# lastz/lastz

Hardware: AMD Instinct MI355X
Metric: Gbp-of-target aligned/sec (whole job, --nogapped HSP path, both strands) (higher is better)
Workload: dtype s32

## Files before the change

include/lzgpu.h:

```cpp
#ifndef LZGPU_H
#define LZGPU_H
#include <stdint.h>
#include <stddef.h>

#ifdef __cplusplus
extern "C" {
#endif

#define LZGPU_MAX_PARTS   16
#define LZGPU_MAX_PROBES  128

#define LZGPU_ERR_NO_DEVICE   (-1)
#define LZGPU_ERR_HIP         (-2)
#define LZGPU_ERR_OOM         (-3)
#define LZGPU_ERR_ARG         (-4)
#define LZGPU_ERR_STATE       (-5)

#define LZGPU_NH_SEED          1
#define LZGPU_NH_SCORE_CLASSES 2
#define LZGPU_NH_HITS_OVERFLOW 3
#define LZGPU_NH_HSP_OVERFLOW  4
#define LZGPU_NH_SIZE          5
#define LZGPU_NH_IDENTICAL     6
#define LZGPU_NH_UNSUPPORTED   7
// ... 158 lines not shown
int lzgpu_reduce_to_chain(const lz_chain_args* a, const lz_segment* segs, uint32_t n, uint32_t** kept, uint32_t* n_kept, int32_t* best);
int lzgpu_reduce_to_chain_batch(const lz_chain_args* a, const lz_segment* const* segs, const uint32_t* n, uint32_t k,
                                uint32_t** kept, uint32_t* n_kept, int32_t* best);

typedef struct lz_counters {
    uint64_t words;
    uint64_t raw_hits;
    uint64_t extensions;
    uint64_t bp_extended;
    uint64_t hsps;
    uint64_t dp_cells;
    uint64_t gapped_extensions;
    uint64_t anchors_extended;
    uint64_t truncated_extensions;
    uint64_t dp_rows;
} lz_counters;
void lzgpu_counters_reset(void);
int  lzgpu_counters_get(lz_counters* out);

void lzgpu_profile_enable(int enable);
void lzgpu_profile_reset(void);
int  lzgpu_profile_get(int n, const char** name, uint64_t* launches, double* total_ms);

int lzgpu_set_hit_capacity(uint64_t max_hits_per_chunk);
int lzgpu_set_hsp_capacity(uint64_t max_candidate_hsps);
int lzgpu_set_dp_slot(uint32_t first_try_traceback_bytes_per_dp);
int lzgpu_set_dp_window(uint32_t max_anchors_speculated_per_round);
int lzgpu_dp_longest(uint64_t out[4], int reset);

int lzgpu_set_bucket_owner(uint32_t n_owners, uint32_t owner);
int lzgpu_last_scan_mode(void);
int lzgpu_set_scan_mode(int min_mode);
int lzgpu_last_hsp_order(uint64_t* out , uint64_t n);

#ifdef __cplusplus
}
#endif
#endif
```

lastz_amd/build.py:

```python
import os
import subprocess
import sys

HERE = os.path.dirname(os.path.abspath(__file__))
CSRC = os.environ.get("LZGPU_CSRC") or os.path.join(HERE, "csrc")
OUT = os.path.join(HERE, "liblzgpu.so")
SOURCES = ["lzgpu_api.hip", "seq_kernels.hip", "table_kernels.hip", "limit_kernels.hip", "mask_kernels.hip", "enum_kernels.hip", "scan_kernels.hip", "exact_kernels.hip", "mismatch_kernels.hip", "filter_kernels.hip", "settle_kernels.hip", "dp_kernels.hip", "dp_kernels_narrow.hip", "window_kernels.hip", "lz_share.hip", "lz_host.cpp", "lz_gapped_host.cpp", "lz_dp_pieces.cpp", "lz_chain_host.cpp"]
FLAGS = ["--offload-arch=gfx950", "-O3", "-std=c++17", "-fPIC", "-Wall", "-Wno-unused-result"] + os.environ.get("LZGPU_CXXFLAGS", "").split()


def _stale(obj, srcs):
    if not os.path.exists(obj):
        return True
    t = os.path.getmtime(obj)
    return any(os.path.getmtime(s) > t for s in srcs)


def build(force=False, verbose=False):
    hipcc = os.environ.get("HIPCC", "/opt/rocm/bin/hipcc")
    tag = os.environ.get("LZGPU_BUILD_TAG", "")
    out = OUT if not tag else os.path.join(HERE, "liblzgpu_%s.so" % tag)
    objdir = os.path.join(HERE, "build" if not tag else "build_" + tag)
    os.makedirs(objdir, exist_ok=True)
    headers = [os.path.join(CSRC, f) for f in os.listdir(CSRC) if f.endswith((".hpp", ".h", ".inc"))]
    headers.append(os.path.join(HERE, "..", "include", "lzgpu.h"))
    objs = []
    procs = []
    for src in SOURCES:
        sp = os.path.join(CSRC, src)
        obj = os.path.join(objdir, src + ".o")
        objs.append(obj)
        if force or _stale(obj, [sp] + headers):
            flags = FLAGS if src.endswith(".hip") else ["-x", "c++"] + [f for f in FLAGS if not f.startswith("--offload")]
            cmd = [hipcc] + flags + ["-c", sp, "-o", obj]
            if verbose:
                print(" ".join(cmd))
            procs.append((src, subprocess.Popen(cmd)))
    for src, p in procs:
        if p.wait() != 0:
            raise RuntimeError(f"hipcc failed on {src}")
# ... 11 lines not shown
```

lastz_amd/csrc/lz_ctx.hpp:

```cpp
#pragma once
#include <hip/hip_runtime.h>
#include <string>
#include <vector>
#include <map>
#include <mutex>
#include "lz_common.hpp"
#include "lz_settings.hpp"
#include "../../include/lzgpu.h"

struct DevBuf {
    void*  p = nullptr;
    size_t cap = 0;
    int ensure(size_t bytes);
    void release();
    template <class T> T* as() const { return (T*)p; }
};

struct KernelTimer {
    struct Pending { int id; hipEvent_t a, b; hipStream_t s; };
    bool enabled = false;
    std::vector<std::string> names;
    std::vector<uint64_t> launches;
    std::vector<double> ms;
    std::vector<Pending> pending;
// ... 60 lines not shown
    DevBuf wctx;
    u64 wctx_gen = 0; uint64_t wctx_code_key = 0;

    std::map<int, SeqSlot> queries;
#define LZ_TEMP_SLOT_B3 (-1000)
    std::mutex slots_m;

    DevBuf cnt, off, pk;
    DevBuf wiv, wsk, wsv;
    DevBuf blk_start;
    std::vector<u64> blk_start_host;
    u32 blk_shift = 0, blk_count = 1;
    u64* pinned = nullptr; size_t pinned_words = 0;
    DevBuf bins;
    DevBuf keys;
    DevBuf keys2;
    DevBuf filter_keep, filter_counts, filter_bases;
    DevBuf bin_base;
    DevBuf hist, hist_part, run_addr;
    DevBuf summ, scan_tasks, scan_ntasks;
    DevBuf lut;
    DevBuf sort_tmp, scan_tmp;
    DevBuf diag_end;
    DevBuf score_tab;
    std::vector<s32> score_sub;
    u8 rowc[256] = { 0 }, colc[256] = { 0 };
    std::vector<s32> lut_m4; s32 lut_xdrop = -1;
    DevBuf cls_t, cls_q, cls_tmp;
    DevBuf win_tab;
    DevBuf match_tmp;
    DevBuf hsp_out, hsp_count;
    DevBuf hsp_mc;
    DevBuf dev_counters;
    DevBuf tb_keys, tb_vals, tb_keys2, tb_vals2;
    DevBuf mask_bits, mask_ranges;
    struct DpBufs { DevBuf jobs, ids, res, tab, tb, rows, ops, ops_off, ops_out, pieces, rings, sel_jobs, sel_res, problems; } dp;
    DevBuf win_jobs, win_scratch, win_out, win_count;
    bool win_attr_set = false;
    bool settle_attr_set = false;
    bool settle_exact_attr_set = false;
    bool settle_mismatch_attr_set = false;
    u64 dp_longest[4] = { 0, 0, 0, 0 };
    u32 dp_slot_tb = 8u << 20;
    u32 dp_window = 0;
    u32 n_owners = 1, owner = 0;
    bool filter_on = false;
    lz_hit_filter filter = {};
    u64 filter_dropped = 0;
    LzSelfDev self = {};
    DevBuf self_sep;
    std::vector<u64> last_order;
    int min_scan_mode = 0;
    int last_scan_mode = -1;
    u64 hit_capacity = (1ull << 31);
    u64 hsp_capacity = (1ull << 24);

    lz_counters counters = {};
    std::mutex counters_m;
    KernelTimer timer;
    KernelTimer dp_timer;

    void release_device_memory()
    {
        DevBuf* all[] = { &wstart, &wpos, &full_wstart, &full_wpos, &wctx, &cnt, &off, &pk, &wiv, &wsk, &wsv, &blk_start, &bins, &keys, &keys2, &filter_keep, &filter_counts, &filter_bases, &bin_base, &hist, &hist_part, &run_addr,
                          &summ, &scan_tasks, &scan_ntasks, &lut, &sort_tmp, &scan_tmp, &diag_end, &score_tab, &cls_t, &cls_q, &cls_tmp, &win_tab, &match_tmp,
                          &hsp_out, &hsp_count, &hsp_mc, &dev_counters, &tb_keys, &tb_vals, &tb_keys2, &tb_vals2, &mask_bits, &mask_ranges, &self_sep,
                          &dp.jobs, &dp.ids, &dp.res, &dp.tab, &dp.tb, &dp.rows, &dp.ops, &dp.ops_off, &dp.ops_out, &dp.pieces, &dp.rings, &dp.sel_jobs, &dp.sel_res, &dp.problems,
                          &win_jobs, &win_scratch, &win_out, &win_count };
        for (DevBuf* b : all) b->release();
        target.release();
        for (auto& kv : queries) kv.second.release();
        queries.clear();
        if (pinned) (void)hipHostFree(pinned);
        pinned = nullptr; pinned_words = 0;
        have_table = false; wctx_gen = 0; wctx_code_key = 0; limit = 0; full_num_words = 0;
        score_sub.clear(); lut_m4.clear(); lut_xdrop = -1;
        win_attr_set = false; settle_attr_set = false; settle_exact_attr_set = false; settle_mismatch_attr_set = false;
    }
};

LzCtx& lz_ctx();
int lz_bind_thread();
int lz_fail(int code, const char* fmt, ...);
#define LZ_HIP(expr) do { hipError_t _e = (expr); if (_e != hipSuccess) \
    return lz_fail(LZGPU_ERR_HIP, "%s:%d %s -> %s", __FILE__, __LINE__, #expr, hipGetErrorString(_e)); } while (0)

struct LzChunk; struct LzLutParams; struct LzExactParams; struct LzMismatchParams; struct LzFilterParams;
#include "lz_tile_runs.hpp"
int lzk_encode(LzCtx& c, const u8* raw, u8* code, u32 len, const u8* cls256_dev, hipStream_t st = nullptr, KernelTimer* timer = nullptr);
int lzk_pack_nibbles(LzCtx& c, const u8* code_alloc, u8* nib, size_t nbytes);
int lzk_pack2(LzCtx& c, const u8* code_base, const u8* raw_base, u32 len, u8* two, u8* spc, u32 nmask, u32* flags256);
int lzk_overlap32(LzCtx& c, const u8* src, u8* dst, size_t nblocks);
int lzk_table_build(LzCtx& c);
int lzk_table_export(LzCtx& c, u32* last_dev, u32* prev_dev, u32 prev_entries);
int lzk_wctx_build(LzCtx& c);
void lz_limit_lift(LzCtx& c);
int lzk_table_limit(LzCtx& c, u32 limit);
int lzk_table_count_distribution(LzCtx& c, std::vector<u32>& count, std::vector<u32>& words);
int lzk_table_mask(LzCtx& c, const lz_interval* iv, u32 n, u32 tlen);
int lzk_count_hits(LzCtx& c, const u8* qcode, u32 lo, u32 hi);
int lzk_scan_counts(LzCtx& c, u32 n);
int lzk_sample_offsets(LzCtx& c, u32 n, u32 stride, u32 ns);
int lzk_fill_hits(LzCtx& c, u32 lo, const LzChunk& ch, u32 n);
int lzk_scan_reserve(LzCtx& c, int mode, u64 max_n);
int lzk_scan_hits(LzCtx& c, int mode, const LzExtendParams& P, const LzLutParams& Q, u64 n);
int lzk_fused_reserve(LzCtx& c, u64 max_n);
int lzk_scan_fused(LzCtx& c, u32 lo, const LzChunk& ch, u32 n, const LzExtendParams& P, const LzLutParams& Q);
int lzk_partition(LzCtx& c, bool tagged, u64 n);
int lzk_hist_scan(LzCtx& c, u64 n);
int lzk_settle(LzCtx& c, const LzExtendParams& P, u64 n, u32 out_cap);
int lzk_hsp_match_counts(LzCtx& c, u32 n_rec, const SeqSlot& q);
int lzk_settle_exact(LzCtx& c, const LzExactParams& P, u64 n, u32 out_cap);
int lzk_settle_mismatch(LzCtx& c, const LzMismatchParams& P, u64 n, u32 out_cap);
int lzk_scan_exact(LzCtx& c, const LzExactParams& P, u64 n);
int lzk_scan_mismatch(LzCtx& c, const LzMismatchParams& P, u64 n);
int lzk_filter_reserve(LzCtx& c, u64 max_n);
int lzk_filter_hits(LzCtx& c, const LzFilterParams& F, u64 n, u64* n_kept);
```

lastz_amd/csrc/lz_settings.hpp:

```cpp
#pragma once
#include <stdlib.h>
#include <string>

struct LzSettings {
    bool hostprof;
    bool gaps;
    std::string timer_only;
    int scan_mode;
    unsigned long long hit_capacity;
    bool fused_scan;
    unsigned task_region_cap;
    unsigned dp_horizon;
    unsigned helper_min_anchors;
    unsigned helpers;
    unsigned batch_threads;
    unsigned chain_threads;
};

struct LzDpSwitches {
    int narrow, repl;
    std::string dump;
    bool prof;
    unsigned window;
};

namespace lz_env {
inline int      flag01(const char* e) { return e ? e[0] == '1' : -1; }
inline unsigned positive(const char* e, unsigned unset) { const int v = e ? atoi(e) : 0; return v > 0 ? (unsigned)v : unset; }
}

inline LzSettings lz_settings_read()
{
    using namespace lz_env;
    LzSettings s;
    s.hostprof = getenv("LZGPU_HOSTPROF") != nullptr;
    s.gaps = getenv("LZGPU_GAPS") != nullptr;
    { const char* e = getenv("LZGPU_TIMER_ONLY"); s.timer_only = e ? e : ""; }
    { const char* e = getenv("LZGPU_SCAN_MODE"); const int v = e ? atoi(e) : -1; s.scan_mode = v >= 0 && v <= 2 ? v : -1; }
    { const char* e = getenv("LZGPU_HIT_CAPACITY"); const long long v = e ? atoll(e) : 0; s.hit_capacity = v >= 1024 && v <= (1ll << 31) ? (unsigned long long)v : 0; }
    { const char* e = getenv("LZGPU_FUSED_SCAN"); s.fused_scan = !(e && atoi(e) == 0); }
    s.task_region_cap = positive(getenv("LZGPU_TASK_REGION_CAP"), 0);
    { const char* e = getenv("LZGPU_DP_HORIZON"); s.dp_horizon = (unsigned)(e ? atoi(e) : 0); }
    { const char* e = getenv("LZGPU_HELPER_MIN_ANCHORS"); s.helper_min_anchors = (unsigned)(e ? atoi(e) : 20000); }
    s.helpers = positive(getenv("LZGPU_HELPERS"), 0);
    s.batch_threads = positive(getenv("LZGPU_BATCH_THREADS"), 64);
    s.chain_threads = positive(getenv("LZGPU_CHAIN_THREADS"), 16);
    return s;
}
inline const LzSettings& lz_settings() { static const LzSettings s = lz_settings_read(); return s; }

inline LzDpSwitches lz_dp_switches()
{
    using namespace lz_env;
    LzDpSwitches d;
    d.narrow = flag01(getenv("LZGPU_DP_NARROW"));
    d.repl = flag01(getenv("LZGPU_DP_REPL"));
    { const char* e = getenv("LZGPU_DPDUMP"); d.dump = e ? e : ""; }
    d.prof = getenv("LZGPU_DPPROF") != nullptr;
    d.window = positive(getenv("LZGPU_DP_WINDOW"), 0);
    return d;
}
```

lastz_amd/csrc/lzgpu_api.hip:

```cpp
#include <hip/hip_runtime.h>
#include <stdarg.h>
#include <stdio.h>
#include <stdlib.h>
#include <string.h>
#include <math.h>
#include <algorithm>
#include <mutex>
#include <thread>
#include <atomic>
#include "lz_ctx.hpp"
#include "lz_host.hpp"
#include "lz_lut.hpp"
#include "lz_exact.hpp"
#include "lz_mismatch.hpp"
#include "lz_filter.hpp"


static LzCtx g_ctx;
void lz_phase_clocks_print();
LzCtx& lz_ctx() { return g_ctx; }

static thread_local std::string t_last_error, t_last_error_out;
static std::mutex g_err_m;
int lz_fail(int code, const char* fmt, ...)
{
    char buf[512];
    va_list ap; va_start(ap, fmt); vsnprintf(buf, sizeof(buf), fmt, ap); va_end(ap);
    t_last_error = buf;
    std::lock_guard<std::mutex> lk(g_err_m);
    g_ctx.last_error = buf;
    return code;
}

int DevBuf::ensure(size_t bytes)
{
    if (bytes <= cap && p) return 0;
    const bool prof = lz_settings().hostprof;
    const auto t0 = std::chrono::steady_clock::now();
    const size_t old = cap;
    if (p) { (void)hipFree(p); p = nullptr; cap = 0; }
    const auto t1 = std::chrono::steady_clock::now();
    size_t want = bytes < 256 ? 256 : bytes;
    if (want >= (64u << 20)) {
        size_t step = (size_t)1 << 22;
        while (step * 32 <= want) step <<= 1;
        want = (want + step - 1) / step * step;
    }
    hipError_t e = hipMalloc(&p, want);
// ... 73 lines not shown
    return t_last_error_out.c_str();
}

extern "C" int lzgpu_probe(void)
{
    int n = 0;
    if (hipGetDeviceCount(&n) != hipSuccess || n <= 0) return lz_fail(LZGPU_ERR_NO_DEVICE, "no HIP device visible");
    hipDeviceProp_t prop;
    if (hipGetDeviceProperties(&prop, 0) != hipSuccess) return lz_fail(LZGPU_ERR_NO_DEVICE, "hipGetDeviceProperties failed");
    if (strncmp(prop.gcnArchName, "gfx950", 6) != 0)
        return lz_fail(LZGPU_ERR_NO_DEVICE, "device 0 is %s, this library is built for gfx950 only", prop.gcnArchName);
    return 0;
}

static int lz_init_locked(int device_index)
{
    if (g_ctx.inited && (device_index < 0 || device_index == g_ctx.device)) return 0;
    if (g_ctx.inited) return lz_fail(LZGPU_ERR_STATE, "already bound to device %d", g_ctx.device);
    int rc = lzgpu_probe();
    if (rc) return rc;
    if (device_index < 0) {
        const char* lr = getenv("LOCAL_RANK");
        device_index = lr ? atoi(lr) : 0;
        int n = 0; (void)hipGetDeviceCount(&n);
        if (n > 0) device_index %= n;
    }
    LZ_HIP(hipSetDevice(device_index));
    { hipDeviceProp_t prop; if (hipGetDeviceProperties(&prop, device_index) == hipSuccess && prop.multiProcessorCount > 0) g_ctx.num_cus = prop.multiProcessorCount; }
    LZ_HIP(hipStreamCreateWithFlags(&g_ctx.stream, hipStreamNonBlocking));
    LZ_HIP(hipStreamCreateWithFlags(&g_ctx.dp_stream, hipStreamNonBlocking));
    const LzSettings& S = lz_settings();
    if (S.scan_mode >= 0) g_ctx.min_scan_mode = S.scan_mode;
    if (S.hit_capacity) g_ctx.hit_capacity = S.hit_capacity;
    g_ctx.device = device_index;
    g_ctx.inited = true;
    return 0;
}

static std::mutex g_init_mutex;
static std::atomic<int> g_async_state{0};
static void lz_wait_async() { while (g_async_state.load(std::memory_order_acquire) == 1) std::this_thread::yield(); }
extern "C" void lzgpu_init_async(int device_index)
{
    int expect = 0;
    if (!g_async_state.compare_exchange_strong(expect, 1)) return;
    atexit(lz_wait_async);
    std::thread([device_index]() {
        { std::lock_guard<std::mutex> lk(g_init_mutex); (void)lz_init_locked(device_index); }
        g_async_state.store(2, std::memory_order_release);
    }).detach();
}
extern "C" int lzgpu_init(int device_index)
{
    lz_wait_async();
    std::lock_guard<std::mutex> lk(g_init_mutex);
    const int rc = lz_init_locked(device_index);
    if (!rc) LZ_HIP(hipSetDevice(g_ctx.device));
    return rc;
}
extern "C" int lzgpu_device_index(void) { return g_ctx.inited ? g_ctx.device : -1; }

extern "C" void lzgpu_shutdown(void)
{
    LzCtx& c = g_ctx;
    if (!c.inited) return;
    (void)hipSetDevice(c.device);
// ... 673 lines not shown
    if ((rc = ss_filter(c, s, nh))) return rc;
    if (nh == 0) return 0;
    std::vector<u64> hk(nh);
    LZ_HIP(hipMemcpyAsync(hk.data(), c.keys.p, (size_t)nh * 8, hipMemcpyDeviceToHost, c.stream));
    LZ_HIP(hipStreamSynchronize(c.stream));
    for (u64 k : hk) { u32 p2 = (u32)k; s.plain.push_back({ p2 + (u32)(k >> 32), p2, s.L, 0 }); }
    return 0;
}

static int ss_finish(LzCtx& c, SeedSearch& s, lz_hsp** out, uint64_t* n_out)
{
    const lz_search_args* a = s.a;
    int rc;
    u64 hc[3] = { 0, 0, 0 }; u32 n_rec = 0;
    LZ_HIP(hipMemcpyAsync(hc, c.dev_counters.p, 24, hipMemcpyDeviceToHost, c.stream));
    LZ_HIP(hipMemcpyAsync(&n_rec, c.hsp_count.p, 4, hipMemcpyDeviceToHost, c.stream));
    LZ_HIP(hipStreamSynchronize(c.stream));
    g_hp.lap(4, "wait for GPU");
    const bool extend = s.extend();
    const s32 K = s.exact() ? 0 : a->hsp_threshold;
    const int entropic = s.exact() ? 0 : a->entropic;
    const bool gpu_counts = extend && n_rec > 0 && n_rec <= s.out_cap;
    if (gpu_counts) {
        if ((rc = c.hsp_mc.ensure((size_t)n_rec * 20))) return rc;
        if ((rc = lzk_hsp_match_counts(c, n_rec, *s.qs))) return rc;
    }
    c.timer.resolve();
    { std::lock_guard<std::mutex> lk(c.counters_m);
      c.counters.words += hc[2]; c.counters.raw_hits += s.total_hits;
      c.counters.extensions += hc[0]; c.counters.bp_extended += hc[1]; }
    if (!extend) return lz_hsps_out(s.plain, out, n_out);
    if (n_rec > s.out_cap) return LZGPU_NH_HSP_OVERFLOW;

    std::vector<LzHspRec> recs(n_rec);
    std::vector<u32> mc;
    if (n_rec) LZ_HIP(hipMemcpyAsync(recs.data(), c.hsp_out.p, (size_t)n_rec * sizeof(LzHspRec), hipMemcpyDeviceToHost, c.stream));
    if (gpu_counts) { mc.resize((size_t)n_rec * 5); LZ_HIP(hipMemcpyAsync(mc.data(), c.hsp_mc.p, (size_t)n_rec * 20, hipMemcpyDeviceToHost, c.stream)); }
    LZ_HIP(hipStreamSynchronize(c.stream));
    c.timer.resolve();
    g_hp.lap(5, "copy candidates");
    std::vector<lz_hsp> fin;
    if ((rc = lzh_finish_hsps(recs.data(), n_rec, c.target.host.data(), s.qhost, c.seed, c.geom.char_to_bits,
                              K, entropic, fin, gpu_counts ? mc.data() : nullptr, &c.last_order)))
        return lz_fail(rc, "internal: candidate HSP is not on a seed hit");
    if ((rc = lz_hsps_out(fin, out, n_out))) return rc;
    { std::lock_guard<std::mutex> lk(c.counters_m); c.counters.hsps += fin.size(); }
    g_hp.lap(6, "host finish (order+entropy)");
    return 0;
}

static int filter_check(LzCtx& c, const int8_t* match_bits)
{
    if (!c.filter_on) return 0;
    const lz_hit_filter& f = c.filter;
    const u32 L = (u32)c.seed.length;
    if (f.positions == 0 || (L < 32 && (f.positions >> L) != 0)) return lz_fail(LZGPU_ERR_ARG, "hit filter: positions %08x of a seed of length %u", f.positions, L);
    if (f.min_matches < 0 || f.min_matches > __builtin_popcount(f.positions))
        return lz_fail(LZGPU_ERR_ARG, "hit filter: %d matches of %d positions", (int)f.min_matches, __builtin_popcount(f.positions));
    if (match_bits && memcmp(match_bits, f.match_bits, 256) != 0)
        return lz_fail(LZGPU_ERR_ARG, "hit filter: the search's match_bits differ from the filter's (a slot holds one set of match codes)");
    if (c.n_owners > 1) return LZGPU_NH_UNSUPPORTED;
    return 0;
}

static int seed_search(const lz_search_args* a, lz_hsp** out, uint64_t* n_out, const int8_t* match_bits = nullptr, u32 mismatches = 0)
{
    LzCtx& c = g_ctx;
    SeedSearch s; s.a = a; s.match_bits = match_bits; s.mismatches = mismatches;
    int rc;
    c.filter_dropped = 0;
    if ((rc = filter_check(c, match_bits))) return rc;
    s.filtered = c.filter_on;
    g_hp.start();
    if ((rc = ss_query(c, s))) return rc;
    if ((rc = ss_classes(c, s))) return rc;
    if (s.qs->len < s.L) return 0;
    if ((rc = ss_count(c, s))) return rc;
    if ((rc = ss_plan(c, s))) return rc;
    if ((rc = ss_scan_mode(c, s))) return rc;
    if ((rc = ss_reserve(c, s))) return rc;
    for (const LzChunk& ch : s.chunks) if ((rc = s.exact() ? ss_chunk_exact(c, s, ch) : a->extend ? ss_chunk(c, s, ch) : ss_chunk_plain(c, s, ch))) return rc;
    g_hp.lap(3, "chunk loop launches");
    return ss_finish(c, s, out, n_out);
}

extern "C" int lzgpu_seed_hit_search(const lz_search_args* a, lz_hsp** out, uint64_t* n_out)
{
    int rc = search_enter(a && out && n_out && a->sub, out, n_out);
    return rc ? rc : seed_search(a, out, n_out);
}

extern "C" int lzgpu_seed_hit_search_exact(const lz_search_args* a, const int8_t match_bits[256], lz_hsp** out, uint64_t* n_out)
{
    int rc = search_enter(a && match_bits && out && n_out, out, n_out); if (rc) return rc;
    if (g_ctx.n_owners > 1) return LZGPU_NH_UNSUPPORTED;
    return seed_search(a, out, n_out, match_bits);
}

extern "C" int lzgpu_seed_hit_search_mismatch(const lz_search_args* a, const int8_t match_bits[256], int32_t max_mismatches, lz_hsp** out, uint64_t* n_out)
{
    int rc = search_enter(a && match_bits && out && n_out, out, n_out); if (rc) return rc;
    if (max_mismatches < 1 || max_mismatches > (int32_t)LZ_MM_MAX) return lz_fail(LZGPU_ERR_ARG, "in seed_hit_search_mismatch(), %d mismatches (1..%u)", (int)max_mismatches, LZ_MM_MAX);
    if (a->hsp_threshold < 1) return lz_fail(LZGPU_ERR_ARG, "in seed_hit_search_mismatch(), length %d", (int)a->hsp_threshold);
// ... 120 lines not shown
    return 0;
}
extern "C" int lzgpu_set_hit_capacity(uint64_t n)
{
    if (n < 1024 || n > (1ull << 31)) return LZGPU_ERR_ARG;
    g_ctx.hit_capacity = n; return 0;
}
extern "C" int lzgpu_set_bucket_owner(uint32_t n_owners, uint32_t owner)
{
    if (n_owners < 1 || n_owners > LZ_DIAG_SIZE || owner >= n_owners) return LZGPU_ERR_ARG;
    g_ctx.n_owners = n_owners; g_ctx.owner = owner;
    return 0;
}
extern "C" int lzgpu_set_hit_filter(const lz_hit_filter* f)
{
    g_ctx.filter_on = f != nullptr;
    if (f) g_ctx.filter = *f;
    return 0;
}
extern "C" int lzgpu_last_filter_dropped(uint64_t* dropped)
{
    if (!dropped) return LZGPU_ERR_ARG;
    *dropped = g_ctx.filter_dropped;
    return 0;
}
extern "C" int lzgpu_last_hsp_order(uint64_t* out, uint64_t n)
{
    if (!out || 2 * n != g_ctx.last_order.size()) return LZGPU_ERR_ARG;
    memcpy(out, g_ctx.last_order.data(), g_ctx.last_order.size() * 8);
    return 0;
}
extern "C" int lzgpu_last_scan_mode(void) { return g_ctx.last_scan_mode; }
extern "C" int lzgpu_set_scan_mode(int min_mode) { if (min_mode < 0 || min_mode > 2) return LZGPU_ERR_ARG; g_ctx.min_scan_mode = min_mode; return 0; }
extern "C" int lzgpu_set_hsp_capacity(uint64_t n) { if (n < 16) return LZGPU_ERR_ARG; g_ctx.hsp_capacity = n; return 0; }
```

lastz_amd/lzgpu.py:

```python
import ctypes as C
import os
import numpy as np

_HERE = os.path.dirname(os.path.abspath(__file__))
LIB_PATH = os.environ.get("LZGPU_LIB") or os.path.join(_HERE, "liblzgpu.so")

MAX_PARTS, MAX_PROBES = 16, 128

NH_REASONS = {1: "SEED", 2: "SCORE_CLASSES", 3: "HITS_OVERFLOW", 4: "HSP_OVERFLOW", 5: "SIZE",
              6: "IDENTICAL", 7: "UNSUPPORTED", 8: "PAIRED_LIMIT"}


class SeedDesc(C.Structure):
    _fields_ = [("length", C.c_int32), ("weight_bits", C.c_int32), ("num_parts", C.c_int32),
                ("shift", C.c_int32 * MAX_PARTS), ("mask", C.c_uint32 * MAX_PARTS),
                ("num_probes", C.c_int32), ("probe_xor", C.c_uint32 * MAX_PROBES)]


class TableGeom(C.Structure):
    _fields_ = [("tlen", C.c_uint32), ("start", C.c_uint32), ("end", C.c_uint32), ("step", C.c_uint32),
                ("num_words", C.c_uint64), ("seed", SeedDesc), ("char_to_bits", C.c_int8 * 256)]


class SearchArgs(C.Structure):
# ... 21 lines not shown


class SelfArgs(C.Structure):
    _fields_ = [("same_strand", C.c_int32), ("band_width", C.c_uint32), ("sep1", C.c_void_p), ("n_sep1", C.c_uint32),
                ("sep2", C.c_void_p), ("n_sep2", C.c_uint32)]


class PosFilter(C.Structure):
    _fields_ = [("t_start", C.c_uint32), ("t_end", C.c_uint32), ("q_start", C.c_uint32), ("q_end", C.c_uint32)]


class HitFilter(C.Structure):
    _fields_ = [("min_matches", C.c_int32), ("max_transversions", C.c_int32), ("positions", C.c_uint32), ("match_bits", C.c_int8 * 256)]


class Counters(C.Structure):
    _fields_ = [("words", C.c_uint64), ("raw_hits", C.c_uint64), ("extensions", C.c_uint64),
                ("bp_extended", C.c_uint64), ("hsps", C.c_uint64), ("dp_cells", C.c_uint64),
                ("gapped_extensions", C.c_uint64), ("anchors_extended", C.c_uint64), ("truncated_extensions", C.c_uint64),
                ("dp_rows", C.c_uint64)]


HSP_DTYPE = np.dtype([("pos1", "<u4"), ("pos2", "<u4"), ("length", "<u4"), ("score", "<i4")])
SEG_DTYPE = np.dtype([("pos1", "<u4"), ("pos2", "<u4"), ("length", "<u4"), ("s", "<i4"), ("id", "<i4")])
ALIGN_DTYPE = np.dtype([("beg1", "<u4"), ("beg2", "<u4"), ("end1", "<u4"), ("end2", "<u4"),
                        ("s", "<i4"), ("script_len", "<u4"), ("script_off", "<u4")])

EXPORTS = ["lzgpu_seed_from_pattern", "lzgpu_probe", "lzgpu_init", "lzgpu_device_index", "lzgpu_init_async", "lzgpu_shutdown", "lzgpu_free",
           "lzgpu_last_error", "lzgpu_table_prepare", "lzgpu_table_export", "lzgpu_table_rebuild", "lzgpu_target_patch", "lzgpu_target_update", "lzgpu_table_mask", "lzgpu_table_num_words",
           "lzgpu_table_geom", "lzgpu_table_adopt", "lzgpu_table_buffers", "lzgpu_table_commit", "lzgpu_table_share", "lzgpu_table_save", "lzgpu_table_load", "lzgpu_table_limit", "lzgpu_table_find_limit", "lzgpu_table_count_distribution", "lzgpu_device_copy",
           "lzgpu_seed_hit_search", "lzgpu_seed_hit_search_self", "lzgpu_seed_hit_search_within", "lzgpu_seed_hit_search_exact", "lzgpu_seed_hit_search_mismatch", "lzgpu_query_upload", "lzgpu_target_upload", "lzgpu_gapped_extend", "lzgpu_gapped_extend_batch", "lzgpu_window_search",
           "lzgpu_counters_reset", "lzgpu_counters_get", "lzgpu_profile_enable", "lzgpu_profile_reset",
           "lzgpu_profile_get", "lzgpu_set_hit_capacity", "lzgpu_set_hsp_capacity", "lzgpu_set_dp_slot", "lzgpu_set_dp_window", "lzgpu_dp_longest",
           "lzgpu_set_bucket_owner", "lzgpu_set_hit_filter", "lzgpu_last_filter_dropped", "lzgpu_last_hsp_order", "lzgpu_last_scan_mode", "lzgpu_set_scan_mode", "lzgpu_reduce_to_chain", "lzgpu_reduce_to_chain_batch"]


class LzGpuError(RuntimeError):
    pass


class NotHandled(Exception):
    def __init__(self, rc):
        super().__init__(f"not handled: {NH_REASONS.get(rc, rc)}")
        self.rc = rc


def _ptr(a):
    return a.ctypes.data_as(C.c_void_p)


class Lib:

    def __init__(self, path=LIB_PATH, prefix="lzgpu_"):
        if not os.path.exists(path):
            raise LzGpuError(f"{path} is missing: run `python -c 'import __graft_entry__ as g; g.build()'`")
        self.L = C.CDLL(path)
        self.px = prefix
        f = self._f
        f("seed_hit_search").argtypes = [C.POINTER(SearchArgs), C.POINTER(C.c_void_p), C.POINTER(C.c_uint64)]
        if prefix == "lzgpu_":
            self.L.lzgpu_seed_hit_search_self.argtypes = [C.POINTER(SearchArgs), C.POINTER(SelfArgs), C.POINTER(C.c_void_p), C.POINTER(C.c_uint64)]
            self.L.lzgpu_seed_hit_search_within.argtypes = [C.POINTER(SearchArgs), C.POINTER(PosFilter), C.POINTER(C.c_void_p), C.POINTER(C.c_uint64)]
            self.L.lzgpu_seed_hit_search_exact.argtypes = [C.POINTER(SearchArgs), C.c_void_p, C.POINTER(C.c_void_p), C.POINTER(C.c_uint64)]
            self.L.lzgpu_seed_hit_search_mismatch.argtypes = [C.POINTER(SearchArgs), C.c_void_p, C.c_int32, C.POINTER(C.c_void_p), C.POINTER(C.c_uint64)]
        f("table_prepare").argtypes = [C.c_void_p, C.c_uint32, C.c_uint32, C.c_uint32, C.c_void_p,
                                       C.POINTER(SeedDesc), C.c_uint32]
        f("set_hit_capacity").argtypes = [C.c_uint64]
# ... 212 lines not shown
    def set_bucket_owner(self, n_owners, owner):
        self._check(self._f("set_bucket_owner")(C.c_uint32(n_owners), C.c_uint32(owner)), "lzgpu_set_bucket_owner")

    def set_hit_filter(self, match_bits=None, min_matches=0, max_transversions=-1, positions=0):
        self.L.lzgpu_set_hit_filter.argtypes = [C.c_void_p]
        if match_bits is None:
            self._check(self.L.lzgpu_set_hit_filter(None), "lzgpu_set_hit_filter")
            return
        f = HitFilter()
        f.min_matches, f.max_transversions, f.positions = min_matches, max_transversions, positions
        mb = np.ascontiguousarray(match_bits, dtype=np.int8)
        assert len(mb) == 256
        C.memmove(f.match_bits, _ptr(mb), 256)
        self._check(self.L.lzgpu_set_hit_filter(C.byref(f)), "lzgpu_set_hit_filter")

    def last_filter_dropped(self):
        n = C.c_uint64()
        self.L.lzgpu_last_filter_dropped.argtypes = [C.POINTER(C.c_uint64)]
        self._check(self.L.lzgpu_last_filter_dropped(C.byref(n)), "lzgpu_last_filter_dropped")
        return int(n.value)

    def table_save(self, path):
        self._check(self.L.lzgpu_table_save(str(path).encode()), "lzgpu_table_save")

    def table_load(self, path):
        self._check(self.L.lzgpu_table_load(str(path).encode()), "lzgpu_table_load")

    def last_scan_mode(self):
        return int(self.L.lzgpu_last_scan_mode())

    def set_scan_mode(self, min_mode):
        self._check(self.L.lzgpu_set_scan_mode(C.c_int(min_mode)), "lzgpu_set_scan_mode")

    def last_hsp_order(self, n):
        out = np.zeros((n, 2), dtype=np.uint64)
        self._check(self._f("last_hsp_order")(_ptr(out), C.c_uint64(n)), "lzgpu_last_hsp_order")
        return out

    def target_upload(self, t):
        t = np.ascontiguousarray(t, dtype=np.uint8)
        self._check(self.L.lzgpu_target_upload(_ptr(t), len(t)), "lzgpu_target_upload")

    def _gapped_args(self, keep, sub, anchors, q=None, slot=-1, gap_open=400, gap_extend=30, ydrop=9400, score_thresh=3000,
                     traceback_bytes=0, reduce=True, sep1=None, sep2=None, strands_differ=False, inhibit_trivial=False,
                     t_off=0, t_len=0, q_off=0, q_len=0, all_bounds=False, no_trim=False, max_paired_bases=0):
        a = GappedArgs()
        a.strands_differ, a.inhibit_trivial = int(strands_differ), int(inhibit_trivial)
        a.all_bounds, a.no_trim, a.max_paired_bases = int(all_bounds), int(no_trim), int(max_paired_bases)
        a.t_off, a.t_len, a.q_off, a.q_len = t_off, t_len, q_off, q_len
        if sep1 is not None:
            sep1 = np.ascontiguousarray(sep1, dtype=np.uint32); a.sep1, a.n_sep1 = sep1.ctypes.data, len(sep1)
        if sep2 is not None:
            sep2 = np.ascontiguousarray(sep2, dtype=np.uint32); a.sep2, a.n_sep2 = sep2.ctypes.data, len(sep2)
        sub = np.ascontiguousarray(sub, dtype=np.int32)
        anchors = np.ascontiguousarray(anchors.copy(), dtype=SEG_DTYPE)
        if q is not None:
            q = np.ascontiguousarray(q, dtype=np.uint8)
            a.query, a.qlen = q.ctypes.data, len(q)
        else:
            a.query, a.qlen = None, self._keep[("qlen", slot)]
        a.query_slot = slot
        a.sub, a.gap_open, a.gap_extend, a.ydrop = sub.ctypes.data, gap_open, gap_extend, ydrop
        a.score_thresh, a.traceback_bytes = score_thresh, traceback_bytes
        a.anchors, a.n_anchors, a.reduce = anchors.ctypes.data, len(anchors), int(reduce)
        keep += [sub, anchors, q, sep1, sep2]
        return a
# ... 126 lines not shown
```

Before: 0.4188.

## Move HSP finish (sort, entropy score, compaction) from host to device

Result: faster. 0.4286, median of 6 (+2.3%).

```diff
diff --git a/include/lzgpu.h b/include/lzgpu.h
--- a/include/lzgpu.h
+++ b/include/lzgpu.h
@@ -214,6 +214,11 @@
 int lzgpu_last_scan_mode(void);
 int lzgpu_set_scan_mode(int min_mode);
 int lzgpu_last_hsp_order(uint64_t* out , uint64_t n);
+#define LZGPU_FINISH_HOST             0
+#define LZGPU_FINISH_DEVICE           1
+#define LZGPU_FINISH_DEVICE_THEN_HOST 2
+int lzgpu_last_finish(void);
+int lzgpu_set_device_finish(int on);
 
 #ifdef __cplusplus
 }
diff --git a/lastz_amd/build.py b/lastz_amd/build.py
--- a/lastz_amd/build.py
+++ b/lastz_amd/build.py
@@ -5,7 +5,7 @@
 HERE = os.path.dirname(os.path.abspath(__file__))
 CSRC = os.environ.get("LZGPU_CSRC") or os.path.join(HERE, "csrc")
 OUT = os.path.join(HERE, "liblzgpu.so")
-SOURCES = ["lzgpu_api.hip", "seq_kernels.hip", "table_kernels.hip", "limit_kernels.hip", "mask_kernels.hip", "enum_kernels.hip", "scan_kernels.hip", "exact_kernels.hip", "mismatch_kernels.hip", "filter_kernels.hip", "settle_kernels.hip", "dp_kernels.hip", "dp_kernels_narrow.hip", "window_kernels.hip", "lz_share.hip", "lz_host.cpp", "lz_gapped_host.cpp", "lz_dp_pieces.cpp", "lz_chain_host.cpp"]
+SOURCES = ["lzgpu_api.hip", "seq_kernels.hip", "table_kernels.hip", "limit_kernels.hip", "mask_kernels.hip", "enum_kernels.hip", "scan_kernels.hip", "exact_kernels.hip", "mismatch_kernels.hip", "filter_kernels.hip", "settle_kernels.hip", "finish_kernels.hip", "dp_kernels.hip", "dp_kernels_narrow.hip", "window_kernels.hip", "lz_share.hip", "lz_host.cpp", "lz_gapped_host.cpp", "lz_dp_pieces.cpp", "lz_chain_host.cpp"]
 FLAGS = ["--offload-arch=gfx950", "-O3", "-std=c++17", "-fPIC", "-Wall", "-Wno-unused-result"] + os.environ.get("LZGPU_CXXFLAGS", "").split()
 
 
diff --git a/lastz_amd/csrc/finish_kernels.hip b/lastz_amd/csrc/finish_kernels.hip
--- /dev/null
+++ b/lastz_amd/csrc/finish_kernels.hip
@@ -0,0 +1,99 @@
+#include <hip/hip_runtime.h>
+#include <rocprim/device/device_merge_sort.hpp>
+#include <rocprim/device/device_scan.hpp>
+#include "lz_ctx.hpp"
+#include "lz_finish.hpp"
+
+#define LZ_FN_TPB 256
+
+__global__ void __launch_bounds__(LZ_FN_TPB)
+k_finish_keys(const LzHspRec* __restrict__ recs, const u32* __restrict__ mc, u32 n, u32 nprobes, LzFinKey* __restrict__ keys, u32* __restrict__ head)
+{
+    const u32 i = blockIdx.x * LZ_FN_TPB + threadIdx.x;
+    if (i >= n) return;
+    u32 probe = mc[5 * (size_t)i + 4];
+    if (probe >= nprobes) { atomicOr(head + 1, LZ_FIN_BAD_PROBE); probe = 0; }
+    keys[i] = lz_fin_key(recs[i].seed_pos1, recs[i].seed_pos2, probe, i);
+}
+
+__global__ void __launch_bounds__(LZ_FN_TPB)
+k_finish_score(const LzHspRec* __restrict__ recs, const u32* __restrict__ mc, const LzFinKey* __restrict__ order, u32 n, s32 K, int entropic,
+               s32* __restrict__ sims, u32* __restrict__ keep, u32* __restrict__ head)
+{
+    const u32 k = blockIdx.x * LZ_FN_TPB + threadIdx.x;
+    if (k >= n) return;
+    const u32 i = order[k].idx;
+    bool unsure;
+    const s32 sim = lz_fin_score(recs[i].score, recs[i].length, mc + 5 * (size_t)i, K, entropic, unsure);
+    if (unsure) atomicOr(head + 1, LZ_FIN_UNSURE);
+    sims[k] = sim;
+    keep[k] = sim >= K ? 1u : 0u;
+}
+
+__global__ void __launch_bounds__(LZ_FN_TPB)
+k_finish_write(const LzHspRec* __restrict__ recs, const LzFinKey* __restrict__ order, const s32* __restrict__ sims, const u32* __restrict__ keep,
+               const u32* __restrict__ place, u32 n, u32* __restrict__ head, lz_hsp* __restrict__ hsps, u64* __restrict__ words)
+{
+    const u32 k = blockIdx.x * LZ_FN_TPB + threadIdx.x;
+    if (k >= n) return;
+    const u32 w = place[k], kp = keep[k];
+    if (k == n - 1) head[0] = w + kp;
+    if (!kp) return;
+    const LzFinKey o = order[k];
+    hsps[w] = lz_fin_hsp(recs[o.idx], sims[k]);
+    words[2 * (size_t)w] = o.hi; words[2 * (size_t)w + 1] = (u64)o.lo;
+}
+
+int lzk_finish_device(LzCtx& c, u32 n_rec, s32 K, int entropic)
+{
+    int rc;
+    const size_t n = n_rec, block = LZ_FIN_HEAD + n * (sizeof(lz_hsp) + 16);
+    if ((rc = c.fin_keys.ensure(n * sizeof(LzFinKey)))) return rc;
+    if ((rc = c.fin_order.ensure(n * sizeof(LzFinKey)))) return rc;
+    if ((rc = c.fin_sims.ensure(n * 4))) return rc;
+    if ((rc = c.fin_keep.ensure(n * 4))) return rc;
+    if ((rc = c.fin_place.ensure(n * 4))) return rc;
+    if ((rc = c.fin_out.ensure(block))) return rc;
+    if (c.fin_stage_cap < block) {
+        if (c.fin_stage) (void)hipHostFree(c.fin_stage);
+        c.fin_stage = nullptr; c.fin_stage_cap = 0;
+        const size_t want = block + block / 2;
+        LZ_HIP(hipHostMalloc(&c.fin_stage, want, hipHostMallocDefault));
+        c.fin_stage_cap = want;
+    }
+    LzFinKey* const keys = c.fin_keys.as<LzFinKey>(); LzFinKey* const order = c.fin_order.as<LzFinKey>();
+    u32* const head = c.fin_out.as<u32>();
+    lz_hsp* const hsps = (lz_hsp*)((u8*)c.fin_out.p + LZ_FIN_HEAD);
+    u64* const words = (u64*)((u8*)c.fin_out.p + LZ_FIN_HEAD + n * sizeof(lz_hsp));
+    const LzHspRec* const recs = c.hsp_out.as<LzHspRec>(); const u32* const mc = c.hsp_mc.as<u32>();
+    const dim3 grid((unsigned)((n + LZ_FN_TPB - 1) / LZ_FN_TPB)), tpb(LZ_FN_TPB);
+
+    size_t sort_bytes = 0, scan_bytes = 0;
+    LZ_HIP(rocprim::merge_sort(nullptr, sort_bytes, keys, order, n, LzFinLess(), c.stream));
+    LZ_HIP(rocprim::exclusive_scan(nullptr, scan_bytes, c.fin_keep.as<u32>(), c.fin_place.as<u32>(), 0u, n, rocprim::plus<u32>(), c.stream));
+    if ((rc = c.sort_tmp.ensure(sort_bytes))) return rc;
+    if ((rc = c.scan_tmp.ensure(scan_bytes))) return rc;
+
+    LZ_HIP(hipMemsetAsync(head, 0, LZ_FIN_HEAD, c.stream));
+    c.timer.begin("k_finish_keys", c.stream);
+    hipLaunchKernelGGL(k_finish_keys, grid, tpb, 0, c.stream, recs, mc, n_rec, (u32)c.seed.nprobes, keys, head);
+    c.timer.end(c.stream);
+    LZ_HIP(hipGetLastError());
+    c.timer.begin("rocprim_sort_finish", c.stream);
+    LZ_HIP(rocprim::merge_sort(c.sort_tmp.p, sort_bytes, keys, order, n, LzFinLess(), c.stream));
+    c.timer.end(c.stream);
+    c.timer.begin("k_finish_score", c.stream);
+    hipLaunchKernelGGL(k_finish_score, grid, tpb, 0, c.stream, recs, mc, order, n_rec, K, entropic, c.fin_sims.as<s32>(), c.fin_keep.as<u32>(), head);
+    c.timer.end(c.stream);
+    LZ_HIP(hipGetLastError());
+    c.timer.begin("rocprim_scan_finish", c.stream);
+    LZ_HIP(rocprim::exclusive_scan(c.scan_tmp.p, scan_bytes, c.fin_keep.as<u32>(), c.fin_place.as<u32>(), 0u, n, rocprim::plus<u32>(), c.stream));
+    c.timer.end(c.stream);
+    c.timer.begin("k_finish_write", c.stream);
+    hipLaunchKernelGGL(k_finish_write, grid, tpb, 0, c.stream, recs, order, c.fin_sims.as<s32>(), c.fin_keep.as<u32>(), c.fin_place.as<u32>(), n_rec,
+                       head, hsps, words);
+    c.timer.end(c.stream);
+    LZ_HIP(hipGetLastError());
+    LZ_HIP(hipMemcpyAsync(c.fin_stage, c.fin_out.p, block, hipMemcpyDeviceToHost, c.stream));
+    return 0;
+}
diff --git a/lastz_amd/csrc/lz_ctx.hpp b/lastz_amd/csrc/lz_ctx.hpp
--- a/lastz_amd/csrc/lz_ctx.hpp
+++ b/lastz_amd/csrc/lz_ctx.hpp
@@ -116,6 +116,9 @@
     DevBuf hsp_out, hsp_count;
     DevBuf hsp_mc;
     DevBuf dev_counters;
+    DevBuf fin_keys, fin_order, fin_sims, fin_keep, fin_place, fin_out;
+#define LZ_FIN_HEAD 16u
+    void* fin_stage = nullptr; size_t fin_stage_cap = 0;
     DevBuf tb_keys, tb_vals, tb_keys2, tb_vals2;
     DevBuf mask_bits, mask_ranges;
     struct DpBufs { DevBuf jobs, ids, res, tab, tb, rows, ops, ops_off, ops_out, pieces, rings, sel_jobs, sel_res, problems; } dp;
@@ -135,6 +138,8 @@
     DevBuf self_sep;
     std::vector<u64> last_order;
     int min_scan_mode = 0;
+    bool device_finish = true;
+    int last_finish = -1;
     int last_scan_mode = -1;
     u64 hit_capacity = (1ull << 31);
     u64 hsp_capacity = (1ull << 24);
@@ -148,7 +153,7 @@
     {
         DevBuf* all[] = { &wstart, &wpos, &full_wstart, &full_wpos, &wctx, &cnt, &off, &pk, &wiv, &wsk, &wsv, &blk_start, &bins, &keys, &keys2, &filter_keep, &filter_counts, &filter_bases, &bin_base, &hist, &hist_part, &run_addr,
                           &summ, &scan_tasks, &scan_ntasks, &lut, &sort_tmp, &scan_tmp, &diag_end, &score_tab, &cls_t, &cls_q, &cls_tmp, &win_tab, &match_tmp,
-                          &hsp_out, &hsp_count, &hsp_mc, &dev_counters, &tb_keys, &tb_vals, &tb_keys2, &tb_vals2, &mask_bits, &mask_ranges, &self_sep,
+                          &hsp_out, &hsp_count, &hsp_mc, &dev_counters, &fin_keys, &fin_order, &fin_sims, &fin_keep, &fin_place, &fin_out, &tb_keys, &tb_vals, &tb_keys2, &tb_vals2, &mask_bits, &mask_ranges, &self_sep,
                           &dp.jobs, &dp.ids, &dp.res, &dp.tab, &dp.tb, &dp.rows, &dp.ops, &dp.ops_off, &dp.ops_out, &dp.pieces, &dp.rings, &dp.sel_jobs, &dp.sel_res, &dp.problems,
                           &win_jobs, &win_scratch, &win_out, &win_count };
         for (DevBuf* b : all) b->release();
@@ -157,6 +162,8 @@
         queries.clear();
         if (pinned) (void)hipHostFree(pinned);
         pinned = nullptr; pinned_words = 0;
+        if (fin_stage) (void)hipHostFree(fin_stage);
+        fin_stage = nullptr; fin_stage_cap = 0;
         have_table = false; wctx_gen = 0; wctx_code_key = 0; limit = 0; full_num_words = 0;
         score_sub.clear(); lut_m4.clear(); lut_xdrop = -1;
         win_attr_set = false; settle_attr_set = false; settle_exact_attr_set = false; settle_mismatch_attr_set = false;
@@ -196,6 +203,7 @@
 int lzk_hsp_match_counts(LzCtx& c, u32 n_rec, const SeqSlot& q);
 int lzk_settle_exact(LzCtx& c, const LzExactParams& P, u64 n, u32 out_cap);
 int lzk_settle_mismatch(LzCtx& c, const LzMismatchParams& P, u64 n, u32 out_cap);
+int lzk_finish_device(LzCtx& c, u32 n_rec, s32 K, int entropic);
 int lzk_scan_exact(LzCtx& c, const LzExactParams& P, u64 n);
 int lzk_scan_mismatch(LzCtx& c, const LzMismatchParams& P, u64 n);
 int lzk_filter_reserve(LzCtx& c, u64 max_n);
diff --git a/lastz_amd/csrc/lz_finish.hpp b/lastz_amd/csrc/lz_finish.hpp
--- /dev/null
+++ b/lastz_amd/csrc/lz_finish.hpp
@@ -0,0 +1,62 @@
+#pragma once
+#include <math.h>
+#include "lz_common.hpp"
+#include "../../include/lzgpu.h"
+
+#define LZ_FIN_REL     (1.0 / 281474976710656.0)
+#define LZ_FIN_DELTA   (1.0 / 140737488355328.0)
+#define LZ_FIN_TAU     (1.0 / 1099511627776.0)
+
+#define LZ_FIN_BAD_PROBE 1u
+#define LZ_FIN_UNSURE    2u
+
+struct LzFinKey { u64 hi; u32 lo, idx; };
+LZ_HD LzFinKey lz_fin_key(u32 seed_pos1, u32 seed_pos2, u32 probe, u32 idx)
+{
+    LzFinKey k; k.hi = ((u64)seed_pos2 << 32) | probe; k.lo = ~seed_pos1; k.idx = idx;
+    return k;
+}
+struct LzFinLess {
+    LZ_HD bool operator()(const LzFinKey& x, const LzFinKey& y) const { return x.hi != y.hi ? x.hi < y.hi : x.lo < y.lo; }
+};
+
+LZ_HD double lz_fin_log(int c, int len, double p) { return c == 0 || c == len ? 0.0 : log(p); }
+LZ_HD double lz_fin_entropy(int cA, int cC, int cG, int cT, int len)
+{
+    double pA = ((double)cA) / ((double)len), pC = ((double)cC) / ((double)len);
+    double pG = ((double)cG) / ((double)len), pT = ((double)cT) / ((double)len);
+    double qA = lz_fin_log(cA, len, pA), qC = lz_fin_log(cC, len, pC);
+    double qG = lz_fin_log(cG, len, pG), qT = lz_fin_log(cT, len, pT);
+    return -(pA * qA + pC * qC + pG * qG + pT * qT) / log(4.0);
+}
+
+LZ_HD bool lz_fin_unsure(s32 sim, double x)
+{
+    if (x == 0.0) return false;
+    if (!(x < 2147483647.0)) return true;
+    const double d = fabs(x - rint(x));
+    return d <= (double)sim * LZ_FIN_TAU;
+}
+
+LZ_HD s32 lz_fin_score(s32 score, u32 length, const u32* mc, s32 K, int entropic, bool& unsure)
+{
+    unsure = false;
+    s32 sim = score;
+    const s32 zero_thresh = K > 0 ? K : 0;
+    if (entropic && sim >= zero_thresh && (s64)sim <= 3 * (s64)K) {
+        const int cA = (int)mc[0], cC = (int)mc[1], cG = (int)mc[2], cT = (int)mc[3];
+        if (cA + cC + cG + cT >= 20) {
+            const double x = sim * lz_fin_entropy(cA, cC, cG, cT, (int)length);
+            unsure = lz_fin_unsure(sim, x);
+            sim = unsure ? 0 : (s32)x;
+        }
+    }
+    return sim;
+}
+
+LZ_HD lz_hsp lz_fin_hsp(const LzHspRec& r, s32 sim)
+{
+    const s32 diag = (s32)r.seed_pos1 - (s32)r.seed_pos2;
+    lz_hsp h; h.pos1 = r.end1; h.pos2 = (u32)((s32)r.end1 - diag); h.length = r.length; h.score = sim;
+    return h;
+}
diff --git a/lastz_amd/csrc/lz_settings.hpp b/lastz_amd/csrc/lz_settings.hpp
--- a/lastz_amd/csrc/lz_settings.hpp
+++ b/lastz_amd/csrc/lz_settings.hpp
@@ -9,6 +9,7 @@
     int scan_mode;
     unsigned long long hit_capacity;
     bool fused_scan;
+    bool device_finish;
     unsigned task_region_cap;
     unsigned dp_horizon;
     unsigned helper_min_anchors;
@@ -39,6 +40,7 @@
     { const char* e = getenv("LZGPU_SCAN_MODE"); const int v = e ? atoi(e) : -1; s.scan_mode = v >= 0 && v <= 2 ? v : -1; }
     { const char* e = getenv("LZGPU_HIT_CAPACITY"); const long long v = e ? atoll(e) : 0; s.hit_capacity = v >= 1024 && v <= (1ll << 31) ? (unsigned long long)v : 0; }
     { const char* e = getenv("LZGPU_FUSED_SCAN"); s.fused_scan = !(e && atoi(e) == 0); }
+    { const char* e = getenv("LZGPU_DEVICE_FINISH"); s.device_finish = !(e && atoi(e) == 0); }
     s.task_region_cap = positive(getenv("LZGPU_TASK_REGION_CAP"), 0);
     { const char* e = getenv("LZGPU_DP_HORIZON"); s.dp_horizon = (unsigned)(e ? atoi(e) : 0); }
     { const char* e = getenv("LZGPU_HELPER_MIN_ANCHORS"); s.helper_min_anchors = (unsigned)(e ? atoi(e) : 20000); }
diff --git a/lastz_amd/csrc/lzgpu_api.hip b/lastz_amd/csrc/lzgpu_api.hip
--- a/lastz_amd/csrc/lzgpu_api.hip
+++ b/lastz_amd/csrc/lzgpu_api.hip
@@ -14,6 +14,7 @@
 #include "lz_exact.hpp"
 #include "lz_mismatch.hpp"
 #include "lz_filter.hpp"
+#include "lz_finish.hpp"
 
 
 static LzCtx g_ctx;
@@ -153,6 +154,7 @@
     const LzSettings& S = lz_settings();
     if (S.scan_mode >= 0) g_ctx.min_scan_mode = S.scan_mode;
     if (S.hit_capacity) g_ctx.hit_capacity = S.hit_capacity;
+    if (!S.device_finish) g_ctx.device_finish = false;
     g_ctx.device = device_index;
     g_ctx.inited = true;
     return 0;
@@ -892,6 +894,32 @@
     if (!extend) return lz_hsps_out(s.plain, out, n_out);
     if (n_rec > s.out_cap) return LZGPU_NH_HSP_OVERFLOW;
 
+    if (gpu_counts && c.device_finish) {
+        if ((rc = lzk_finish_device(c, n_rec, K, entropic))) return rc;
+        g_hp.lap(9, "device finish: launches");
+        LZ_HIP(hipStreamSynchronize(c.stream));
+        c.timer.resolve();
+        g_hp.lap(10, "device finish: wait");
+        const u32* head = (const u32*)c.fin_stage;
+        const u32 n_fin = head[0], flags = head[1];
+        if (flags & LZ_FIN_BAD_PROBE) return lz_fail(LZGPU_ERR_STATE, "internal: candidate HSP is not on a seed hit");
+        if (n_fin > n_rec) return lz_fail(LZGPU_ERR_STATE, "internal: the finish kept %u of %u candidates", n_fin, n_rec);
+        if (!(flags & LZ_FIN_UNSURE)) {
+            lz_hsp* res = (lz_hsp*)malloc((n_fin ? n_fin : 1) * sizeof(lz_hsp));
+            if (!res) return lz_fail(LZGPU_ERR_OOM, "host malloc failed");
+            const u8* body = (const u8*)c.fin_stage + LZ_FIN_HEAD;
+            memcpy(res, body, (size_t)n_fin * sizeof(lz_hsp));
+            const u64* words = (const u64*)(body + (size_t)n_rec * sizeof(lz_hsp));
+            c.last_order.assign(words, words + 2 * (size_t)n_fin);
+            *out = res; *n_out = n_fin;
+            { std::lock_guard<std::mutex> lk(c.counters_m); c.counters.hsps += n_fin; }
+            c.last_finish = LZGPU_FINISH_DEVICE;
+            g_hp.lap(11, "device finish: copy out");
+            return 0;
+        }
+        c.last_finish = LZGPU_FINISH_DEVICE_THEN_HOST;
+    }
+
     std::vector<LzHspRec> recs(n_rec);
     std::vector<u32> mc;
     if (n_rec) LZ_HIP(hipMemcpyAsync(recs.data(), c.hsp_out.p, (size_t)n_rec * sizeof(LzHspRec), hipMemcpyDeviceToHost, c.stream));
@@ -929,6 +957,7 @@
     SeedSearch s; s.a = a; s.match_bits = match_bits; s.mismatches = mismatches;
     int rc;
     c.filter_dropped = 0;
+    c.last_finish = LZGPU_FINISH_HOST;
     if ((rc = filter_check(c, match_bits))) return rc;
     s.filtered = c.filter_on;
     g_hp.start();
@@ -1115,4 +1144,6 @@
 }
 extern "C" int lzgpu_last_scan_mode(void) { return g_ctx.last_scan_mode; }
 extern "C" int lzgpu_set_scan_mode(int min_mode) { if (min_mode < 0 || min_mode > 2) return LZGPU_ERR_ARG; g_ctx.min_scan_mode = min_mode; return 0; }
+extern "C" int lzgpu_last_finish(void) { return g_ctx.last_finish; }
+extern "C" int lzgpu_set_device_finish(int on) { if (on != 0 && on != 1) return LZGPU_ERR_ARG; g_ctx.device_finish = on != 0; return 0; }
 extern "C" int lzgpu_set_hsp_capacity(uint64_t n) { if (n < 16) return LZGPU_ERR_ARG; g_ctx.hsp_capacity = n; return 0; }
diff --git a/lastz_amd/lzgpu.py b/lastz_amd/lzgpu.py
--- a/lastz_amd/lzgpu.py
+++ b/lastz_amd/lzgpu.py
@@ -77,7 +77,7 @@
            "lzgpu_seed_hit_search", "lzgpu_seed_hit_search_self", "lzgpu_seed_hit_search_within", "lzgpu_seed_hit_search_exact", "lzgpu_seed_hit_search_mismatch", "lzgpu_query_upload", "lzgpu_target_upload", "lzgpu_gapped_extend", "lzgpu_gapped_extend_batch", "lzgpu_window_search",
            "lzgpu_counters_reset", "lzgpu_counters_get", "lzgpu_profile_enable", "lzgpu_profile_reset",
            "lzgpu_profile_get", "lzgpu_set_hit_capacity", "lzgpu_set_hsp_capacity", "lzgpu_set_dp_slot", "lzgpu_set_dp_window", "lzgpu_dp_longest",
-           "lzgpu_set_bucket_owner", "lzgpu_set_hit_filter", "lzgpu_last_filter_dropped", "lzgpu_last_hsp_order", "lzgpu_last_scan_mode", "lzgpu_set_scan_mode", "lzgpu_reduce_to_chain", "lzgpu_reduce_to_chain_batch"]
+           "lzgpu_set_bucket_owner", "lzgpu_set_hit_filter", "lzgpu_last_filter_dropped", "lzgpu_last_hsp_order", "lzgpu_last_scan_mode", "lzgpu_set_scan_mode", "lzgpu_last_finish", "lzgpu_set_device_finish", "lzgpu_reduce_to_chain", "lzgpu_reduce_to_chain_batch"]
 
 
 class LzGpuError(RuntimeError):
@@ -356,6 +356,12 @@
     def set_scan_mode(self, min_mode):
         self._check(self.L.lzgpu_set_scan_mode(C.c_int(min_mode)), "lzgpu_set_scan_mode")
 
+    def last_finish(self):
+        return int(self.L.lzgpu_last_finish())
+
+    def set_device_finish(self, on):
+        self._check(self.L.lzgpu_set_device_finish(C.c_int(1 if on else 0)), "lzgpu_set_device_finish")
+
     def last_hsp_order(self, n):
         out = np.zeros((n, 2), dtype=np.uint64)
         self._check(self._f("last_hsp_order")(_ptr(out), C.c_uint64(n)), "lzgpu_last_hsp_order")
```
